# andreaskoepf/faster-rcnn.torch

Hardware: AMD Instinct MI355X
Metric: images/sec (vgg_small 800x450 fwd+bwd) (higher is better)
Workload: dtype f32 (conv / Linear(13824,1024) operands as 2 x fp16 split planes: 22 significand bits, 3 MFMA partial products; fp32 accumulate)

## Files before the change

faster-rcnn.torch_amd/csrc/amax.h:

```cpp
#pragma once
#include <hip/hip_runtime.h>

#include "kernels.h"

namespace frcnn {

__device__ __forceinline__ void amax_store_block(float m, float* rec) {
  __shared__ float amax_part[16];
#pragma unroll
  for (int o = 32; o > 0; o >>= 1) m = fmaxf(m, __shfl_xor(m, o));
  if ((threadIdx.x & 63) == 0) amax_part[threadIdx.x >> 6] = m;
  __syncthreads();
  if (threadIdx.x == 0) {
    const int nw = (blockDim.x + 63) >> 6;
    for (int i = 1; i < nw; ++i) m = fmaxf(m, amax_part[i]);
    rec[1 + blockIdx.x] = m;
    if (blockIdx.x == 0) rec[0] = __builtin_bit_cast(float, (int)gridDim.x);
  }
}

__device__ __forceinline__ float amax_load_block(const float* __restrict__ rec) {
  __shared__ float amax_all[16];
  const int n = __builtin_bit_cast(int, rec[0]);
  float m = 0.f;
  for (int i = threadIdx.x; i < n; i += blockDim.x) m = fmaxf(m, rec[1 + i]);
#pragma unroll
  for (int o = 32; o > 0; o >>= 1) m = fmaxf(m, __shfl_xor(m, o));
  if ((threadIdx.x & 63) == 0) amax_all[threadIdx.x >> 6] = m;
  __syncthreads();
  const int nw = (blockDim.x + 63) >> 6;
  m = amax_all[0];
  for (int i = 1; i < nw; ++i) m = fmaxf(m, amax_all[i]);
  __syncthreads();
  return m;
}

}
```

faster-rcnn.torch_amd/csrc/cnet.hip:

```cpp
#include "kernels.h"

namespace frcnn {

#define BN_EPS 1e-5
#define BN_MOM 0.1

#define BN_CB 16
#define BN_RG 64
template <int CB = BN_CB, int RG = BN_RG>
__device__ __forceinline__ double bn_reduce(double v, double* sh, int tx, int ty) {
  sh[ty * CB + tx] = v;
  __syncthreads();
  for (int stride = RG / 2; stride > 0; stride >>= 1) {
    if (ty < stride) sh[ty * CB + tx] += sh[(ty + stride) * CB + tx];
    __syncthreads();
  }
  const double s = sh[tx];
  __syncthreads();
  return s;
}
template <int NV>
__device__ __forceinline__ void fb_reduce(double (&v)[NV], double* sh, int tx, int ty) {
  const int tid = ty * 4 + tx, lane = tid & 63, wave = tid >> 6;
#pragma unroll
// ... 230 lines not shown
      FR_LAUNCH(KC_ELEMWISE, 0, total * 16.0, s, cnet_act_forward_flat_kernel<true>, dim3(grid), dim3(256), 0, x, src, total, n, lin, slope,
                mask, inv_keep, p, seed, post);
    else
      FR_LAUNCH(KC_ELEMWISE, 0, total * 16.0, s, cnet_act_forward_flat_kernel<false>, dim3(grid), dim3(256), 0, x, src, total, n, lin, slope,
                mask, inv_keep, p, seed, post);
    FR_LAUNCH_CHECK();
    return FRCNN_OK;
  }
  if (gen)
    FR_LAUNCH(KC_ELEMWISE, 0, (double)R * n * 20.0, s, cnet_act_forward_kernel<true>, dim3(cdiv(n, FB_CB)), dim3(FB_CB, FB_RG), 0, x,
              src, R, n, gamma, beta, running, training, lin, xhat, invstd, pre, slope, mask, inv_keep, p, seed, post);
  else
    FR_LAUNCH(KC_ELEMWISE, 0, (double)R * n * 20.0, s, cnet_act_forward_kernel<false>, dim3(cdiv(n, FB_CB)), dim3(FB_CB, FB_RG), 0, x,
              src, R, n, gamma, beta, running, training, lin, xhat, invstd, pre, slope, mask, inv_keep, p, seed, post);
  FR_LAUNCH_CHECK();
  return FRCNN_OK;
}

__global__ __launch_bounds__(1024) void cnet_act_bn_backward_kernel(const float* __restrict__ gy, GemmFold src,
                                                                    const float* __restrict__ pre, const float* __restrict__ xhat,
                                                                    const float* __restrict__ invstd, const float* __restrict__ gamma,
                                                                    const float* slope, const float* __restrict__ mask, float inv_keep,
                                                                    int R, int n, int training, float* __restrict__ gx, float* ggamma,
                                                                    float* gbeta, float* gslope, float* part) {
  __shared__ double sh[FB_RG * FB_CB];
  __shared__ float shs[16];
  const int tx = threadIdx.x, ty = threadIdx.y;
  const int j = blockIdx.x * FB_CB + tx;
  const bool ok = j < n;
  const size_t total = (size_t)R * n;
  const float a = *slope;
  double sg = 0.0, sgx = 0.0;
  float sa = 0.f;
  const bool keep = R <= FB_RG * FB_KEEP;
  float tv[FB_KEEP], xh[FB_KEEP];
  auto first = [&](size_t idx, float& t, float& xhv) {
    float g = fold_value(gy, src, total, idx, j);
    if (mask) g = g * (mask[idx] * inv_keep);
    const float xv = pre[idx];
    t = g;
    if (!(xv > 0.f)) { t = a * g; sa += xv * g; }
    xhv = xhat[idx];
    sg += t;
    sgx += (double)t * xhv;
  };
  if (ok && keep) {
#pragma unroll
// ... 2 lines not shown
      if (ty + i * FB_RG < R) first((size_t)(ty + i * FB_RG) * n + j, tv[i], xh[i]);
    }
  } else if (ok) {
    for (int r = ty; r < R; r += FB_RG) {
      const size_t idx = (size_t)r * n + j;
      float t, xhv;
      first(idx, t, xhv);
      gx[idx] = t;
    }
  }
  { double t[2] = {sg, sgx}; fb_reduce(t, sh, tx, ty); sg = t[0]; sgx = t[1]; }
  {
    const int tid = ty * FB_CB + tx;
#pragma unroll
    for (int o = 32; o > 0; o >>= 1) sa += __shfl_down(sa, o, 64);
    if ((tid & 63) == 0) shs[tid >> 6] = sa;
    __syncthreads();
    if (tid == 0) {
      float t = 0.f;
      for (int i = 0; i < 16; ++i) t += shs[i];
      if (part) part[blockIdx.x] = t; else unsafeAtomicAdd(gslope, t);
    }
  }
  if (!ok) return;
  if (ty == 0) {
    ggamma[j] = (float)((double)ggamma[j] + sgx);
    gbeta[j] = (float)((double)gbeta[j] + sg);
  }
  const double is = invstd[j], gm = gamma[j];
  auto second = [&](size_t idx, double g, double xhv) {
    const double v = training ? (g - sg / R - xhv * sgx / R) * gm * is : g * gm * is;
    gx[idx] = (float)v;
  };
  if (keep) {
#pragma unroll
    for (int i = 0; i < FB_KEEP; ++i)
      if (ty + i * FB_RG < R) second((size_t)(ty + i * FB_RG) * n + j, tv[i], xh[i]);
  } else {
    for (int r = ty; r < R; r += FB_RG) {
      const size_t idx = (size_t)r * n + j;
      second(idx, gx[idx], xhat[idx]);
    }
  }
}
__global__ void slope_fold_kernel(const float* __restrict__ part, int n, float* gslope);
int cnet_act_bn_backward(const float* gy, GemmFold src, const float* pre, const float* xhat, const float* invstd,
                         const float* gamma, const float* slope, const float* mask, float inv_keep, int R, int n, int training,
                         float* gx, float* ggamma, float* gbeta, float* gslope, hipStream_t s) {
  const int grid = cdiv(n, FB_CB);
  float* part = nullptr;
  if (deterministic()) FR_TRY(det_workspace(s, (size_t)grid, &part));
  FR_LAUNCH(KC_ELEMWISE, 0, (double)R * n * 28.0, s, cnet_act_bn_backward_kernel, dim3(grid), dim3(FB_CB, FB_RG), 0, gy, src, pre, xhat,
            invstd, gamma, slope, mask, inv_keep, R, n, training, gx, ggamma, gbeta, gslope, part);
  if (part) FR_LAUNCH(KC_ELEMWISE, 0, grid * 4.0, s, slope_fold_kernel, dim3(1), dim3(1), 0, (const float*)part, grid, gslope);
  FR_LAUNCH_CHECK();
  return FRCNN_OK;
}

template <bool GEN>
__global__ void prelu_dropout_forward_kernel(const float* __restrict__ x, long n, const float* slope,
                                             float* __restrict__ mask, float inv_keep, float p,
                                             unsigned long long seed, float* __restrict__ y) {
  const float a = *slope;
  for (long i = (long)blockIdx.x * blockDim.x + threadIdx.x; i < n; i += (long)gridDim.x * blockDim.x) {
    float v = x[i];
    v = v > 0.f ? v : a * v;
    if (GEN) {
      const float mk = frcnn_keep_mask(seed, (unsigned long long)i, p);
      mask[i] = mk;
      v = v * (mk * inv_keep);
    } else if (mask) {
      v = v * (mask[i] * inv_keep);
    }
    y[i] = v;
  }
}
// ... 340 lines not shown
```

faster-rcnn.torch_amd/csrc/kernels.h:

```cpp
#pragma once
#include <algorithm>

#include "common.h"

namespace frcnn {

int conv_cc(int k);
int conv_mpad(int M);
size_t conv_pack_floats(int Kchan, int M, int k);
int conv_pack_weights(const float* w, int O, int C, int k, float* wf, float* wd, hipStream_t s);
struct PackJob { long w_off; long total; float* dst; int O, C, k, mode, Mpad, blk_begin, nblk; };
PackJob conv_pack_job(long w_off, int O, int C, int k, int mode, float* dst);
int conv_pack_assign_blocks(PackJob* jobs, int njobs, int total_blocks);
int conv_pack_weights_multi(const float* weights, const PackJob* jobs_dev, int njobs, int grid, hipStream_t s);

enum { OUT_STORE = 0, OUT_ADD = 1 };
struct IgemmPool { float* out; unsigned char* idx; const float* slope; const float* scale; float* amax = nullptr; };
int conv_igemm(const float* in, int Cin, int H, int W, const float* in_slope, const float* in_scale,
               const float* wp, const float* bias, int M, int k, int pad, float* out, int out_mode,
               double algo_flops, hipStream_t s, int ws_slot = 0,
               const IgemmPool* pool = nullptr, bool* pool_fused = nullptr);

void set_split_bf16(int on);
int get_split_bf16();
// ... 159 lines not shown
int roi_windows(const double* rect, const long long* pick, int k, const int* layers, int nlayers, int fmH, int fmW, int* wins,
                hipStream_t s);
int detect_post(const int* cls, const float* conf, const float* bbox, const double* rect, const long long* pick, int R,
                int bgclass, double min_conf, float* bb, int* kc, int* keep_row, double* r2, int* K_dev, hipStream_t s);
int detect_gather(const long long* wpick, const int* nwin_dev, int cap, const int* keep_row, const int* kc, const float* bb,
                  const double* r2, const long long* pick, const float* mp, const double* rect, const int* midx, double* rec,
                  hipStream_t s);

int bn_forward(const float* x, int R, int n, const float* gamma, const float* beta, float* running,
               int training, float* xhat, float* invstd, float* y, hipStream_t s);
int bn_backward(const float* gy, const float* xhat, const float* invstd, const float* gamma, int R,
                int n, int training, float* gx, float* ggamma, float* gbeta, hipStream_t s);
int prelu_dropout_forward(const float* x, long n, const float* slope, const float* mask, float inv_keep,
                          float* y, hipStream_t s);
int prelu_dropout_forward_gen(const float* x, long n, const float* slope, float* mask_out, float p,
                              unsigned long long seed, float* y, hipStream_t s);
int prelu_dropout_backward(const float* gy, const float* x, long n, const float* slope,
                           const float* mask, float inv_keep, float* gx, float* gslope, hipStream_t s);
int cnet_act_forward(const float* x, GemmFold src, int R, int n, const float* gamma, const float* beta, float* running,
                     int training, float* lin, float* xhat, float* invstd, float* pre, const float* slope, float* mask, bool gen,
                     float inv_keep, float p, unsigned long long seed, float* post, hipStream_t s);
int cnet_act_bn_backward(const float* gy, GemmFold src, const float* pre, const float* xhat, const float* invstd,
                         const float* gamma, const float* slope, const float* mask, float inv_keep, int R, int n, int training,
                         float* gx, float* ggamma, float* gbeta, float* gslope, hipStream_t s);
bool cnet_heads_fused_eligible(int nf, int nc);
int cnet_heads_forward(const float* x, int R, int nf, const float* Wb, const float* bb, const float* Wc, const float* bc, int nc,
                       float* bbox_out, float* logits, float* lsm, float* cls_out, hipStream_t s);
struct HeadsPostAct {
  const float* pre = nullptr;
  const float* mask = nullptr;
  float inv_keep = 1.f;
  const float* slope = nullptr;
  float* gslope = nullptr;
};
int cnet_heads_backward(const float* g_bbox, const float* g_cls, const float* lsm, int R, int nf, const float* Wb, const float* Wc,
                        int nc, float* glog, float* gfeat, hipStream_t s, const HeadsPostAct* post = nullptr);
int log_softmax_rows_fold(const float* x, GemmFold src, int R, int n, float* y, float* y2, hipStream_t s);
int dropout_mask(float* mask, long n, float p, unsigned long long seed, hipStream_t s);
struct DropoutJobs { float* ptr[8]; int C[8]; float p[8]; unsigned long long seed[8]; int n; };
int dropout_channel_masks(const DropoutJobs& j, hipStream_t s);
int log_softmax_rows(const float* x, int R, int n, float* y, hipStream_t s);
int cnet_losses(float* crout, const float* crtarget, const float* ccout, const float* cctarget, int R,
                int npos, int ncls, float* crdelta, float* ccdelta, double* loss2, hipStream_t s);
int log_softmax_backward(const float* gy, const float* lsm, int R, int n, float* gx, hipStream_t s);
int cnet_decode(const float* cls_lsm, int R, int ncls, int* cls_out, float* conf_out, hipStream_t s);

int image_rgb2yuv(const float* rgb, float* yuv, int H, int W, hipStream_t s);
// ... 16 lines not shown
```

faster-rcnn.torch_amd/csrc/net.cpp:

```cpp
#include <array>
#include <vector>
#include <cmath>
#include <cstring>

#include "kernels.h"

namespace frcnn {

static const int HEAD_OUT = 18;
static const int SPARSE_MAX_POS = 512;

struct DevBuf {
  void* p = nullptr;
  size_t bytes = 0;
  bool owned = true;
  void view(void* ptr, size_t n) { p = ptr; bytes = n; owned = false; }
  int ensure(size_t need) {
    if (need <= bytes) return FRCNN_OK;
    if (p && owned) (void)hipFree(p);
    owned = true;
    p = nullptr; bytes = 0;
    FR_HIP(hipMalloc(&p, need + 64));
    bytes = need;
    return FRCNN_OK;
// ... 36 lines not shown
  DevBuf delta;
  const int* sp_pos = nullptr;
  int sp_count = -1;
  DevBuf spD, spHX, spHY, spGH, spCol, spDX;
  DevBuf spOut, spSlab;
  hipStream_t stream = nullptr;
  hipEvent_t done = nullptr;
  hipEvent_t gin_done = nullptr;
  bool gin_recorded = false;
};

struct ClsLayer {
  int in, n;
  bool bn;
  float p_drop;
  long w_off, b_off, bnw_off, bnb_off, a_off;
  DevBuf lin, pre, post, xhat, invstd, mask, g;
  DevBuf gin;
  DevBuf xp, xpT, gp, gpT;
  int x_form = 0;
  DevBuf am;
  const float* am_w_of = nullptr;
  long am_w_gen = -1;
};

}

using namespace frcnn;

static int g_drop_compact = -1;
static int drop_compact_on() {
  if (g_drop_compact < 0) g_drop_compact = getenv("FRCNN_DROP_COMPACT") ? (atoi(getenv("FRCNN_DROP_COMPACT")) != 0) : 1;
  return g_drop_compact;
}
static int pool_stream(int slot, hipStream_t* out) {
  static hipStream_t pool[8] = {};
  if (!pool[slot]) FR_HIP(hipStreamCreateWithFlags(&pool[slot], hipStreamNonBlocking));
  *out = pool[slot];
  return FRCNN_OK;
}

static int g_sparse_heads = -1;
static int sparse_heads_on() {
  if (g_sparse_heads < 0) g_sparse_heads = getenv("FRCNN_SPARSE_HEADS") ? (atoi(getenv("FRCNN_SPARSE_HEADS")) != 0) : 1;
  return g_sparse_heads;
}
static int g_static_weights = 0;
static long g_static_gen = 0;

struct frcnn_model {
  frcnn_model_desc d;
  std::vector<Conv> convs;
  std::vector<Block> blocks;
  std::vector<Head> heads;
  std::vector<ClsLayer> cls;
  long pnet_params = 0, total_params = 0;
  long bbox_w_off = 0, bbox_b_off = 0, clsw_off = 0, clsb_off = 0;
  int H = 0, W = 0;
  int training = 0;
  DevBuf delta_last;
  DevBuf zero_arena;
  size_t delta_bytes = 0, gpool_bytes = 0;
  DevBuf pack_jobs;
  DevBuf x3_jobs;
  DevBuf amax, amax_ws, amax_jobs;
  int n_amax = 0, n_amax_jobs = 0, amax_grid = 0;
  float* rec(int id) const { return (float*)amax.p + (size_t)id * AMAX_REC; }
  bool f16_packed = false;
  long eval_packs_gen = -1;
  const float* eval_packs_w = nullptr;
  int n_x3_all = 0, n_x3_fwd = 0, x3_grid_all = 0, x3_grid_fwd = 0;
  int n_pack_fwd = 0, n_pack_all = 0, n_pack_heads = 0, pack_grid_fwd = 0, pack_grid_all = 0, pack_grid_heads = 0;
  bool head_packs_fresh = false;
  struct PackGroup { int pk_off = 0, pk_n = 0, pk_grid = 0, am_off = 0, am_n = 0, am_grid = 0, x3_off = 0, x3_off16 = 0, x3_n = 0, x3_grid = 0; };
  std::vector<PackGroup> groups;
  unsigned fresh_mask = 0;
  const float* fresh_w = nullptr;
  bool fresh_f16 = false;
  static const int DC_RING = 4;
  char* dc_pin = nullptr; DevBuf dc_dev; size_t dc_slot_bytes = 0, dc_idx_off = 0; unsigned dc_step = 0;
  hipEvent_t dc_ev[DC_RING] = {};
  std::vector<PackXJob> x3_host, x3_host16;
  std::vector<int> x3_conv;
  DevBuf dbg_expand;
  std::vector<hipEvent_t> block_rd_ev;
  hipStream_t side = nullptr;
  hipStream_t cw = nullptr;
  hipEvent_t cw_fork = nullptr, cw_done = nullptr;
  bool cw_pending = false;
  std::vector<hipEvent_t> cw_ev;
// ... 235 lines not shown
      }
      m->pk_bb_off = (int)both.size(); m->pk_bb_n = (int)gj.size();
      m->pk_bb_grid = gj.empty() ? 0 : conv_pack_assign_blocks(gj.data(), m->pk_bb_n, 512);
      both.insert(both.end(), gj.begin(), gj.end());
    }
    FR_TRY(m->pack_jobs.ensure(both.size() * sizeof(PackJob)));
    FR_HIP(hipMemcpy(m->pack_jobs.p, both.data(), both.size() * sizeof(PackJob), hipMemcpyHostToDevice));
  }
  {
    {
      int n = 0;
      for (auto& c : m->convs) { c.am = n; n += 3; }
      for (auto& hd : m->heads) { hd.c3.am = n; n += 3; }
      for (auto& b : m->blocks) b.am = n++;
      m->n_amax = n;
      FR_TRY(m->amax.ensure((size_t)n * AMAX_REC * 4));
      FR_TRY(m->amax_ws.ensure((size_t)n * 4));
      std::vector<AmaxJob> aj;
      auto addw = [&](Conv& c) {
        if (c.x_f || c.x_d) aj.push_back(AmaxJob{c.w_off, (long)c.Cout * c.Cin * c.k * c.k, m->rec(c.am + 2), 0});
      };
      for (auto& c : m->convs) addw(c);
      for (auto& hd : m->heads) addw(hd.c3);
      m->n_amax_jobs = (int)aj.size();
      m->amax_grid = tensor_absmax_assign_blocks(aj.data(), m->n_amax_jobs);
      FR_CHECK(m->amax_grid >= 0, "ensure_shapes: a weight tensor is too large for its magnitude record");
      {
        std::vector<AmaxJob> gj;
        for (auto& c : m->convs)
          if (c.x_f || c.x_d) gj.push_back(AmaxJob{c.w_off, (long)c.Cout * c.Cin * c.k * c.k, m->rec(c.am + 2), 0});
        m->am_bb_off = (int)aj.size(); m->am_bb_n = (int)gj.size();
        m->am_bb_grid = gj.empty() ? 0 : tensor_absmax_assign_blocks(gj.data(), m->am_bb_n);
        aj.insert(aj.end(), gj.begin(), gj.end());
      }
      for (size_t g = 0; g <= m->blocks.size(); ++g) {
        std::vector<AmaxJob> gj;
        auto addg = [&](Conv& c) {
          if (c.x_f || c.x_d) gj.push_back(AmaxJob{c.w_off, (long)c.Cout * c.Cin * c.k * c.k, m->rec(c.am + 2), 0});
        };
        if (g < m->blocks.size()) { for (auto& c : m->convs) if (c.block == (int)g) addg(c); }
        else for (auto& hd : m->heads) addg(hd.c3);
        auto& G = m->groups[g];
        G.am_off = (int)aj.size(); G.am_n = (int)gj.size();
        G.am_grid = gj.empty() ? 0 : tensor_absmax_assign_blocks(gj.data(), G.am_n);
        FR_CHECK(G.am_grid >= 0, "ensure_shapes: a weight tensor is too large for its magnitude record");
        aj.insert(aj.end(), gj.begin(), gj.end());
      }
      if (!aj.empty()) {
        FR_TRY(m->amax_jobs.ensure(aj.size() * sizeof(AmaxJob)));
        FR_HIP(hipMemcpy(m->amax_jobs.p, aj.data(), aj.size() * sizeof(AmaxJob), hipMemcpyHostToDevice));
      }
    }
    std::vector<PackXJob> all, fwd, all16, fwd16;
// ... 94 lines not shown
  frcnn_model* m = new frcnn_model();
  m->d = *desc;
  build_layout(m);
  *out = m;
  return FRCNN_OK;
}

int frcnn_model_destroy(frcnn_model* m) {
  if (!m) return FRCNN_OK;
  auto rel = [](Conv& c) { c.wf.release(); c.wd.release(); c.wx.release(); c.wxd.release(); c.x.release(); c.gx.release(); };
  for (auto& c : m->convs) rel(c);
  for (auto& b : m->blocks) { b.scale.release(); b.pooled.release(); b.gpooled.release(); b.pidx.release(); b.dc_bias.release(); }
  if (m->dc_pin) (void)hipHostFree(m->dc_pin);
  for (auto e : m->dc_ev) if (e) (void)hipEventDestroy(e);
  m->dc_dev.release(); m->dbg_expand.release();
  for (auto& h : m->heads) {
    rel(h.c3); rel(h.c1); h.delta.release(); h.spOut.release(); h.spSlab.release();
    h.spD.release(); h.spHX.release(); h.spHY.release(); h.spGH.release(); h.spCol.release(); h.spDX.release();
  }
  for (auto& l : m->cls) {
    l.lin.release(); l.pre.release(); l.post.release(); l.xhat.release(); l.invstd.release();
    l.mask.release(); l.g.release(); l.xp.release(); l.xpT.release(); l.gp.release(); l.gpT.release(); l.am.release();
  }
  m->img.release(); m->wg_ws.release(); m->wg_ws_first.release(); m->pack_jobs.release(); m->x3_jobs.release(); m->zero_arena.release(); m->amax.release(); m->amax_ws.release(); m->amax_jobs.release();
  for (auto e : m->fork_ev) (void)hipEventDestroy(e);
  for (auto& h : m->heads) {
    if (h.done) (void)hipEventDestroy(h.done);
    if (h.gin_done) (void)hipEventDestroy(h.gin_done);
  }
  if (m->chain_ev) (void)hipEventDestroy(m->chain_ev);
  if (m->join_ev) (void)hipEventDestroy(m->join_ev);
  if (m->bwd_ev) (void)hipEventDestroy(m->bwd_ev);
  if (m->heads_gin_ev) (void)hipEventDestroy(m->heads_gin_ev);
  if (m->upd_ev) (void)hipEventDestroy(m->upd_ev);
  if (m->upd_join_ev) (void)hipEventDestroy(m->upd_join_ev);
  for (auto e : m->block_rd_ev) (void)hipEventDestroy(e);
  for (auto e : m->cw_ev) (void)hipEventDestroy(e);
  if (m->cw_fork) (void)hipEventDestroy(m->cw_fork);
  if (m->cw_done) (void)hipEventDestroy(m->cw_done);
  if (m->loss_ev) (void)hipEventDestroy(m->loss_ev);
  for (auto e : m->block_ev) (void)hipEventDestroy(e);
  m->delta_last.release(); m->feat_g.release(); m->logits.release(); m->lsm.release(); m->glog.release();
  m->gtmp.release();
  delete m;
  return FRCNN_OK;
}

// ... 304 lines not shown
  async_heads = async_heads && use_side && training;
  m->heads_deferred = async_heads && sparse_heads_on() && !deterministic() && m->heads.size() <= 4;
  m->heads_sparse_fwd = false; m->heads_gin = false;
  m->last_w = w;
  if (use_side && !m->heads_deferred) { FR_TRY(ensure_side(m)); FR_TRY(ensure_head_streams(m)); }
  DropoutJobs dj;
  dj.n = 0;
  for (size_t b = 0; b < m->blocks.size(); ++b) {
    Block& blk = m->blocks[b];
    if (!blk.has_drop) continue;
    int C = m->d.filters[b];
    if (!training) {
      FR_TRY(fill_value(blk.scale.f(), C, 1.0f - blk.p_drop, s));
    } else if (drop_masks && drop_masks[b]) {
      FR_HIP(hipMemcpyAsync(blk.scale.p, drop_masks[b], (size_t)C * 4, hipMemcpyDeviceToDevice, s));
    } else {
      dj.ptr[dj.n] = blk.scale.f(); dj.C[dj.n] = C; dj.p[dj.n] = blk.p_drop; dj.seed[dj.n] = seed * 131 + b;
      ++dj.n;
    }
  }
  FR_TRY(dropout_channel_masks(dj, s));
  FR_TRY(plan_compact(m, training, drop_masks, seed));
  m->head_packs_fresh = false;
  const bool f16 = get_x3_f16() && m->n_amax_jobs > 0;
  const bool reuse = !training && g_static_weights && m->eval_packs_gen == g_static_gen && m->eval_packs_w == w && m->f16_packed == f16;
  m->f16_packed = f16;
  const bool fresh = training && !m->groups.empty() && m->fresh_mask == (1u << m->groups.size()) - 1 && m->fresh_w == w && m->fresh_f16 == f16 &&
                     !any_compact(m);
  m->fresh_mask = 0;
  if (!reuse && !fresh) {
    static const bool skip_on = !(getenv("FRCNN_HEAD_PACK_SKIP") && atoi(getenv("FRCNN_HEAD_PACK_SKIP")) == 0);
    const bool skip_heads = skip_on && training && m->heads_deferred && any_compact(m) && m->am_bb_n > 0;
    m->head_x3_fresh = !skip_heads;
    if (training && skip_heads) {
      if (m->pk_bb_n) FR_TRY(conv_pack_weights_multi(w, (const PackJob*)m->pack_jobs.p + m->pk_bb_off, m->pk_bb_n, m->pk_bb_grid, s));
    } else if (training)
      FR_TRY(conv_pack_weights_multi(w, (const PackJob*)m->pack_jobs.p, m->n_pack_all, m->pack_grid_all, s));
    else
      FR_TRY(conv_pack_weights_multi(w, (const PackJob*)m->pack_jobs.p + m->n_pack_all, m->n_pack_fwd, m->pack_grid_fwd, s));
    const PackXJob* xjobs = (const PackXJob*)m->x3_jobs.p + (f16 ? m->n_x3_all + m->n_x3_fwd : 0);
    if (f16 && skip_heads)
      FR_TRY(tensor_absmax_multi(w, (const AmaxJob*)m->amax_jobs.p + m->am_bb_off, m->am_bb_n, m->am_bb_grid, s));
    else if (f16)
      FR_TRY(tensor_absmax_multi(w, (const AmaxJob*)m->amax_jobs.p, m->n_amax_jobs, m->amax_grid, s));
    if (training && any_compact(m))
      FR_TRY(pack_compact(m, w, f16, s));
    else if (training)
      FR_TRY(conv_x3_pack_multi(w, xjobs, m->n_x3_all, m->x3_grid_all, s));
    else
      FR_TRY(conv_x3_pack_multi(w, xjobs + m->n_x3_all, m->n_x3_fwd, m->x3_grid_fwd, s));
  }
  m->eval_packs_gen = training ? -1 : g_static_gen;
  m->eval_packs_w = w;
  FR_TRY(m->img.ensure((size_t)3 * H * W * 4));
  FR_HIP(hipMemcpyAsync(m->img.p, img, (size_t)3 * H * W * 4, hipMemcpyDeviceToDevice, s));
  const float* cur = m->img.f();
  const float* cur_slope = nullptr;
  const float* cur_scale = nullptr;
  const float* cur_am = nullptr;
  for (size_t b = 0; b < m->blocks.size(); ++b) {
    Block& blk = m->blocks[b];
    bool pooled_in_conv = false;
    for (int st = 0; st < blk.nconv; ++st) {
      Conv& c = m->convs[blk.first_conv + st];
      const bool last = st == blk.nconv - 1;
      IgemmPool pl = {blk.pooled.f(), (unsigned char*)blk.pidx.p, w + c.a_off,
                      (st == 0 && blk.has_drop) ? blk.scale.f() : nullptr, f16 ? m->rec(blk.am) : nullptr};
// ... 100 lines not shown
    } break;
    case 4: {
      FR_CHECK(index >= 0 && index < (int)m->blocks.size() && m->H > 0 && m->blocks[index].has_drop, "debug_buffer: block %d has no dropout", index);
      const Block& k = m->blocks[index]; b = &k.scale; n = (size_t)m->d.filters[index] * 4;
    } break;
    case 1: {
      FR_CHECK(index >= 0 && index < (int)m->blocks.size() && m->H > 0, "debug_buffer: block %d (after a forward pass)", index);
      const Block& k = m->blocks[index]; b = &k.pidx; n = (size_t)m->d.filters[index] * k.Hp * k.Wp;
    } break;
    case 2: {
      FR_CHECK(index >= 0 && index < (int)m->heads.size() && m->H > 0, "debug_buffer: anchor net %d (after a forward pass)", index);
      const Conv& c = m->heads[index].c3; b = &c.x; n = (size_t)c.Cout * c.Ho * c.Wo * 4;
      if ((m->heads_sparse_fwd || m->heads_deferred) && m->last_w) {
        FR_HIP(hipDeviceSynchronize());
        if (!m->head_x3_fresh) { FR_TRY(refresh_group(m, m->last_w, (int)m->blocks.size(), nullptr)); m->head_x3_fresh = true; }
        FR_TRY(head_forward(m, m->heads[index], m->last_w, nullptr, 0));
        FR_HIP(hipDeviceSynchronize());
      }
    } break;
    case 3: {
      FR_CHECK(index >= 0 && index < (int)m->cls.size() && m->R > 0, "debug_buffer: classification layer %d (after frcnn_cnet_forward)", index);
      const ClsLayer& L = m->cls[index]; b = L.bn ? &L.pre : &L.lin; n = (size_t)m->R * L.n * 4;
    } break;
    default: FR_CHECK(false, "debug_buffer: unknown kind %d", kind);
  }
  FR_CHECK(b->p && b->bytes >= n, "debug_buffer: buffer not allocated yet");
  *ptr = b->p; *bytes = (long long)n;
  return FRCNN_OK;
}

int frcnn_pnet_delta(frcnn_model* m, int i, float** ptr) {
  FR_CHECK(m->H > 0, "pnet_delta: call frcnn_pnet_forward first");
  FR_CHECK(i >= 1 && i <= (int)m->heads.size() + 1, "pnet_delta: index %d out of range", i);
  *ptr = i <= (int)m->heads.size() ? m->heads[i - 1].delta.f() : m->delta_last.f();
  return FRCNN_OK;
}

int frcnn_pnet_set_sparse_deltas(frcnn_model* m, int head, const int* positions, int count) {
  FR_CHECK(head >= 1 && head <= (int)m->heads.size(), "pnet_set_sparse_deltas: head %d out of range", head);
  m->heads[head - 1].sp_pos = positions;
  m->heads[head - 1].sp_count = count;
  return FRCNN_OK;
}

int frcnn_pnet_zero_deltas(frcnn_model* m, void* stream) {
  FR_CHECK(m->H > 0, "pnet_zero_deltas: call frcnn_pnet_forward first");
// ... 288 lines not shown
}

int frcnn_pnet_wait_heads_done(frcnn_model* m, void* stream) {
  FR_CHECK(m->block_ev_valid, "pnet_wait_heads_done: call frcnn_pnet_backward first");
  for (auto& h : m->heads)
    if (h.stream && h.done) FR_HIP(hipStreamWaitEvent(S(stream), h.done, 0));
  if (m->side) {
    FR_TRY(ensure_update_stream(m));
    FR_TRY(chain(m->side, S(stream), m->upd_ev));
  }
  return FRCNN_OK;
}

int frcnn_pnet_wait_block_done(frcnn_model* m, int block, void* stream) {
  FR_CHECK(block >= 1 && block <= (int)m->blocks.size(), "pnet_wait_block_done: block %d out of range", block);
  FR_CHECK(m->update_armed && m->block_ev_valid && (size_t)block <= m->block_ev.size() && (size_t)block <= m->block_rd_ev.size(),
           "pnet_wait_block_done: call frcnn_model_update_stream before the pass and frcnn_pnet_backward first");
  FR_HIP(hipStreamWaitEvent(S(stream), m->block_ev[block - 1], 0));
  FR_HIP(hipStreamWaitEvent(S(stream), m->block_rd_ev[block - 1], 0));
  return FRCNN_OK;
}

static int refresh_group(frcnn_model* m, const float* w, int group, hipStream_t s) {
  const bool f16 = get_x3_f16() && m->n_amax_jobs > 0;
  const frcnn_model::PackGroup& G = m->groups[group];
  if (G.pk_n) FR_TRY(conv_pack_weights_multi(w, (const PackJob*)m->pack_jobs.p + G.pk_off, G.pk_n, G.pk_grid, s));
  if (f16 && G.am_n) FR_TRY(tensor_absmax_multi(w, (const AmaxJob*)m->amax_jobs.p + G.am_off, G.am_n, G.am_grid, s));
  if (G.x3_n) FR_TRY(conv_x3_pack_multi(w, (const PackXJob*)m->x3_jobs.p + (f16 ? G.x3_off16 : G.x3_off), G.x3_n, G.x3_grid, s));
  return FRCNN_OK;
}
int frcnn_pnet_refresh_packs(frcnn_model* m, const float* w, int group, void* stream) {
  FR_CHECK(m->H > 0, "pnet_refresh_packs: call frcnn_pnet_forward first");
  FR_CHECK(group >= 0 && group < (int)m->groups.size(), "pnet_refresh_packs: group %d out of range", group);
  const bool f16 = get_x3_f16() && m->n_amax_jobs > 0;
  if (m->fresh_mask && (m->fresh_w != w || m->fresh_f16 != f16)) m->fresh_mask = 0;
  FR_TRY(refresh_group(m, w, group, S(stream)));
  if (group == (int)m->blocks.size()) m->head_x3_fresh = true;
  m->fresh_mask |= 1u << group; m->fresh_w = w; m->fresh_f16 = f16;
  return FRCNN_OK;
}

int frcnn_pnet_invalidate_packs(frcnn_model* m) {
  m->fresh_mask = 0;
  return FRCNN_OK;
}

int frcnn_pnet_wait_block_gradients(frcnn_model* m, int block, void* stream) {
  FR_CHECK(block >= 1 && block <= (int)m->blocks.size(), "pnet_wait_block_gradients: block %d out of range", block);
  FR_CHECK(m->block_ev_valid && (size_t)block <= m->block_ev.size(), "pnet_wait_block_gradients: call frcnn_pnet_backward first");
  FR_HIP(hipStreamWaitEvent(S(stream), m->block_ev[block - 1], 0));
  return FRCNN_OK;
}

static int record_block_read(frcnn_model* m, int b, hipStream_t s) {
  if (!m->update_armed) return FRCNN_OK;
  while (m->block_rd_ev.size() < m->blocks.size()) {
    hipEvent_t e;
// ... 189 lines not shown
    if (L.x_form & 1) FR_TRY(L.xp.ensure((size_t)3 * R * L.in * 2));
    if (L.x_form & 2) FR_TRY(L.gp.ensure((size_t)3 * R * L.n * 2));
    if (L.x_form & 4) { FR_TRY(L.xpT.ensure((size_t)3 * L.in * Rp * 2)); FR_TRY(L.gpT.ensure((size_t)3 * L.n * Rp * 2)); }
    if (L.x_form & 7) FR_TRY(L.am.ensure((size_t)5 * AMAX_REC * 4));
  }
  int nc = m->d.class_count + 1;
  int nf = m->cls.empty() ? m->D : m->cls.back().n;
  FR_TRY(m->feat_g.ensure((size_t)R * nf * 4));
  FR_TRY(m->logits.ensure((size_t)R * nc * 4));
  FR_TRY(m->lsm.ensure((size_t)R * nc * 4));
  FR_TRY(m->glog.ensure((size_t)R * nc * 4));
  return FRCNN_OK;
}

int frcnn_cnet_forward(frcnn_model* m, const float* weights, const float* x, int R, int training,
                       const float* const* drop_masks, unsigned long long seed, float* bn_running,
                       float* bbox_out, float* cls_out, void* stream) {
  hipStream_t s = S(stream);
  FR_CHECK(R > 0, "cnet_forward: empty batch");
  FR_TRY(cw_join(m, s));
  FR_TRY(ensure_cnet(m, R));
  m->R = R; m->cnet_x = x; m->training = training;
  const float* w = weights;
  const float* cur = x;
  float* bnr = bn_running;
  for (size_t l = 0; l < m->cls.size(); ++l) {
    ClsLayer& L = m->cls[l];
    GemmFold fold;
    GemmFold* defer = cnet_fuse() ? &fold : nullptr;
    if ((L.x_form & 3) && gemm_f16_on()) {
      float* rw = L.am.f() + 2 * AMAX_REC;
      const bool have = !training && g_static_weights && L.am_w_gen == g_static_gen && L.am_w_of == w;
      if (!have) FR_TRY(tensor_absmax(w + L.w_off, (long)L.n * L.in, rw, s));
      L.am_w_of = w; L.am_w_gen = training ? -1 : g_static_gen;
    } else {
      L.am_w_of = nullptr;
    }
    if ((L.x_form & 1) && gemm_f16_on()) {
      float* rx = L.am.f();
      FR_TRY(tensor_absmax(cur, (long)R * L.in, rx, s));
      FR_TRY(split_planes(cur, R, L.in, L.xp.p, nullptr, s, rx));
      FR_TRY(linear_x_forward(L.xp.p, R, L.in, w + L.w_off, w + L.b_off, L.n, L.lin.f(), s, 0, defer, rx, rx + 2 * AMAX_REC));
    } else if (L.x_form & 1) {
      FR_TRY(split_planes(cur, R, L.in, L.xp.p, nullptr, s));
      FR_TRY(linear_x_forward(L.xp.p, R, L.in, w + L.w_off, w + L.b_off, L.n, L.lin.f(), s, 0, defer));
    } else {
      FR_TRY(gemm_f32(cur, L.in, 1, w + L.w_off, 1, L.in, L.lin.f(), L.n, R, L.n, L.in, OUT_STORE, w + L.b_off, s, 0, defer));
    }
    if (L.bn) FR_CHECK(training || bnr, "cnet_forward: evaluate mode needs bn_running");
    const float* mask = nullptr;
    float inv_keep = 1.f;
    bool draw = false;
    if (training && L.p_drop > 0.f) {
      inv_keep = 1.0f / (1.0f - L.p_drop);
      if (drop_masks && drop_masks[l])
        FR_HIP(hipMemcpyAsync(L.mask.p, drop_masks[l], (size_t)R * L.n * 4, hipMemcpyDeviceToDevice, s));
      else
        draw = true;
      mask = L.mask.f();
    }
    if (defer) {
      FR_TRY(cnet_act_forward(L.lin.f(), fold, R, L.n, L.bn ? w + L.bnw_off : nullptr, L.bn ? w + L.bnb_off : nullptr, L.bn ? bnr : nullptr,
                              training, L.lin.f(), L.xhat.f(), L.invstd.f(), L.pre.f(), w + L.a_off, const_cast<float*>(mask), draw,
                              inv_keep, L.p_drop, seed * 977 + l + 17, L.post.f(), s));
      if (L.bn && bnr) bnr += 2 * L.n;
// ... 74 lines not shown
      post.slope = w + T.a_off; post.gslope = grad + T.a_off;
      dst = T.g.f();
      top_act_done = true;
    }
    FR_TRY(cnet_heads_backward(g_bbox, g_cls, m->lsm.f(), R, nf, w + m->bbox_w_off, w + m->clsw_off, nc, m->glog.f(), dst, s,
                               top_act_done ? &post : nullptr));
    FR_TRY(fork());
  } else {
    FR_TRY(log_softmax_backward(g_cls, m->lsm.f(), R, nc, m->glog.f(), s));
    FR_TRY(fork());
    FR_TRY(gemm_f32(g_bbox, 4, 1, w + m->bbox_w_off, nf, 1, m->feat_g.f(), nf, R, nf, 4, OUT_STORE, nullptr, s));
    FR_TRY(gemm_f32(m->glog.f(), nc, 1, w + m->clsw_off, nf, 1, m->feat_g.f(), nf, R, nf, nc, OUT_ADD, nullptr, s));
  }
  FR_TRY(gemm_f32(g_bbox, 1, 4, feat, nf, 1, grad + m->bbox_w_off, nf, 4, nf, R, OUT_ADD, nullptr, ws, wslot));
  FR_TRY(channel_sum_cols(g_bbox, R, 4, grad + m->bbox_b_off, ws));
  FR_TRY(gemm_f32(m->glog.f(), 1, nc, feat, nf, 1, grad + m->clsw_off, nf, nc, nf, R, OUT_ADD, nullptr, ws, wslot));
  FR_TRY(channel_sum_cols(m->glog.f(), R, nc, grad + m->clsb_off, ws));
  const float* g = m->feat_g.f();
  GemmFold gfold;
  for (int l = (int)m->cls.size() - 1; l >= 0; --l) {
    ClsLayer& L = m->cls[l];
    const float* pre = L.bn ? L.pre.f() : L.lin.f();
    const bool drop = m->training && L.p_drop > 0.f;
    if (top_act_done && l == (int)m->cls.size() - 1) {
    } else if (L.bn && cnet_fuse()) {
      FR_TRY(cnet_act_bn_backward(g, gfold, pre, L.xhat.f(), L.invstd.f(), w + L.bnw_off, w + L.a_off, drop ? L.mask.f() : nullptr,
                                  drop ? 1.0f / (1.0f - L.p_drop) : 1.f, R, L.n, m->training, L.g.f(), grad + L.bnw_off,
                                  grad + L.bnb_off, grad + L.a_off, s));
    } else {
      FR_TRY(prelu_dropout_backward(g, pre, (long)R * L.n, w + L.a_off, drop ? L.mask.f() : nullptr,
                                    drop ? 1.0f / (1.0f - L.p_drop) : 1.f, L.g.f(), grad + L.a_off, s));
      if (L.bn)
        FR_TRY(bn_backward(L.g.f(), L.xhat.f(), L.invstd.f(), w + L.bnw_off, R, L.n, m->training, L.g.f(),
                           grad + L.bnw_off, grad + L.bnb_off, s));
    }
    gfold = GemmFold{};
    GemmFold* gdefer = (cnet_fuse() && async && l > 0 && m->cls[l - 1].bn) ? &gfold : nullptr;
    FR_TRY(fork());
    const float* in = l == 0 ? m->cnet_x : m->cls[l - 1].post.f();
    float* gin = l == 0 ? gx : L.gin.f();
    const bool xw = (L.x_form & 4) != 0, xd = (L.x_form & 2) != 0 && gin;
    if (xd && gemm_f16_on() && L.am_w_of == w) {
      float* rg = L.am.f() + AMAX_REC;
      FR_TRY(tensor_absmax(L.g.f(), (long)R * L.n, rg, s));
      FR_TRY(split_planes(L.g.f(), R, L.n, L.gp.p, nullptr, s, rg));
      FR_TRY(linear_x_dgrad(L.gp.p, R, L.n, w + L.w_off, L.in, gin, OUT_STORE, s, 0, gdefer, rg, L.am.f() + 2 * AMAX_REC));
    } else if (xd) {
      FR_TRY(split_planes(L.g.f(), R, L.n, L.gp.p, nullptr, s));
      FR_TRY(linear_x_dgrad(L.gp.p, R, L.n, w + L.w_off, L.in, gin, OUT_STORE, s, 0, gdefer));
    } else if (gin) {
      FR_TRY(gemm_f32(L.g.f(), L.n, 1, w + L.w_off, L.in, 1, gin, L.in, R, L.in, L.n, OUT_STORE, nullptr, s, 0, gdefer));
    }
    static const bool wgrad_f16 = !(getenv("FRCNN_GEMM_WGRAD_F16") && atoi(getenv("FRCNN_GEMM_WGRAD_F16")) == 0);
    if (xw && wgrad_f16 && gemm_f16_on() && L.am.bytes >= (size_t)5 * AMAX_REC * 4) {
      float *rgT = L.am.f() + 3 * AMAX_REC, *rxT = L.am.f() + 4 * AMAX_REC;
      FR_TRY(tensor_absmax(L.g.f(), (long)R * L.n, rgT, ws));
      if ((L.x_form & 1) && L.am_w_of == w) rxT = L.am.f();
      else FR_TRY(tensor_absmax(in, (long)R * L.in, rxT, ws));
      FR_TRY(split_planes(L.g.f(), R, L.n, nullptr, L.gpT.p, ws, rgT));
      FR_TRY(split_planes(in, R, L.in, nullptr, L.xpT.p, ws, rxT));
      FR_TRY(linear_x_wgrad(L.gpT.p, L.xpT.p, R, L.n, L.in, grad + L.w_off, ws, wslot, rgT, rxT));
    } else if (xw) {
      FR_TRY(split_planes(L.g.f(), R, L.n, nullptr, L.gpT.p, ws));
      FR_TRY(split_planes(in, R, L.in, nullptr, L.xpT.p, ws));
      FR_TRY(linear_x_wgrad(L.gpT.p, L.xpT.p, R, L.n, L.in, grad + L.w_off, ws, wslot));
    } else {
      FR_TRY(gemm_f32(L.g.f(), 1, L.n, in, L.in, 1, grad + L.w_off, L.in, L.n, L.in, R, OUT_ADD, nullptr, ws, wslot));
    }
    FR_TRY(channel_sum_cols(L.g.f(), R, L.n, grad + L.b_off, ws));
    g = gin;
  }
  if (m->cls.empty() && gx) FR_HIP(hipMemcpyAsync(gx, g, (size_t)R * m->D * 4, hipMemcpyDeviceToDevice, s));
  if (async) {
    FR_HIP(hipEventRecord(m->cw_done, ws));
    m->cw_pending = true;
  }
  return FRCNN_OK;
}

// ... 2 lines not shown
```

Measured before the change: 515.7.

## Fuse gradient absmax into BN backward and batch cnet weight absmax with pack jobs

The fused activation/BN backward kernel now also records each block's gradient magnitude maximum. The separate tensor_absmax passes on the classifier gradient (for dgrad and wgrad) can then be dropped, and the wgrad path reuses that record. Classifier weight absmax jobs are appended to the existing multi-tensor absmax launch at the start of a step, so the forward pass can skip its per-layer weight absmax launches. This saves several small kernel launches and extra reads of the gradient and weights, at the cost of more bookkeeping state and a cross-stream dependency on the head-of-step record.

```diff
diff --git a/faster-rcnn.torch_amd/csrc/amax.h b/faster-rcnn.torch_amd/csrc/amax.h
--- a/faster-rcnn.torch_amd/csrc/amax.h
+++ b/faster-rcnn.torch_amd/csrc/amax.h
@@ -5,19 +5,20 @@
 
 namespace frcnn {
 
-__device__ __forceinline__ void amax_store_block(float m, float* rec) {
+__device__ __forceinline__ void amax_store_block(float m, float* rec, int tid, int nthreads) {
   __shared__ float amax_part[16];
 #pragma unroll
   for (int o = 32; o > 0; o >>= 1) m = fmaxf(m, __shfl_xor(m, o));
-  if ((threadIdx.x & 63) == 0) amax_part[threadIdx.x >> 6] = m;
+  if ((tid & 63) == 0) amax_part[tid >> 6] = m;
   __syncthreads();
-  if (threadIdx.x == 0) {
-    const int nw = (blockDim.x + 63) >> 6;
+  if (tid == 0) {
+    const int nw = (nthreads + 63) >> 6;
     for (int i = 1; i < nw; ++i) m = fmaxf(m, amax_part[i]);
     rec[1 + blockIdx.x] = m;
     if (blockIdx.x == 0) rec[0] = __builtin_bit_cast(float, (int)gridDim.x);
   }
 }
+__device__ __forceinline__ void amax_store_block(float m, float* rec) { amax_store_block(m, rec, threadIdx.x, blockDim.x); }
 
 __device__ __forceinline__ float amax_load_block(const float* __restrict__ rec) {
   __shared__ float amax_all[16];
diff --git a/faster-rcnn.torch_amd/csrc/cnet.hip b/faster-rcnn.torch_amd/csrc/cnet.hip
--- a/faster-rcnn.torch_amd/csrc/cnet.hip
+++ b/faster-rcnn.torch_amd/csrc/cnet.hip
@@ -1,3 +1,4 @@
+#include "amax.h"
 #include "kernels.h"
 
 namespace frcnn {
@@ -276,7 +277,7 @@
                                                                     const float* __restrict__ invstd, const float* __restrict__ gamma,
                                                                     const float* slope, const float* __restrict__ mask, float inv_keep,
                                                                     int R, int n, int training, float* __restrict__ gx, float* ggamma,
-                                                                    float* gbeta, float* gslope, float* part) {
+                                                                    float* gbeta, float* gslope, float* part, float* amax_rec) {
   __shared__ double sh[FB_RG * FB_CB];
   __shared__ float shs[16];
   const int tx = threadIdx.x, ty = threadIdx.y;
@@ -325,36 +326,41 @@
       if (part) part[blockIdx.x] = t; else unsafeAtomicAdd(gslope, t);
     }
   }
-  if (!ok) return;
-  if (ty == 0) {
-    ggamma[j] = (float)((double)ggamma[j] + sgx);
-    gbeta[j] = (float)((double)gbeta[j] + sg);
-  }
-  const double is = invstd[j], gm = gamma[j];
-  auto second = [&](size_t idx, double g, double xhv) {
-    const double v = training ? (g - sg / R - xhv * sgx / R) * gm * is : g * gm * is;
-    gx[idx] = (float)v;
-  };
-  if (keep) {
-#pragma unroll
-    for (int i = 0; i < FB_KEEP; ++i)
-      if (ty + i * FB_RG < R) second((size_t)(ty + i * FB_RG) * n + j, tv[i], xh[i]);
-  } else {
-    for (int r = ty; r < R; r += FB_RG) {
-      const size_t idx = (size_t)r * n + j;
-      second(idx, gx[idx], xhat[idx]);
-    }
-  }
+  float am = 0.f;
+  if (ok) {
+    if (ty == 0) {
+      ggamma[j] = (float)((double)ggamma[j] + sgx);
+      gbeta[j] = (float)((double)gbeta[j] + sg);
+    }
+    const double is = invstd[j], gm = gamma[j];
+    auto second = [&](size_t idx, double g, double xhv) {
+      const double v = training ? (g - sg / R - xhv * sgx / R) * gm * is : g * gm * is;
+      gx[idx] = (float)v;
+      am = fmaxf(am, fabsf((float)v));
+    };
+    if (keep) {
+#pragma unroll
+      for (int i = 0; i < FB_KEEP; ++i)
+        if (ty + i * FB_RG < R) second((size_t)(ty + i * FB_RG) * n + j, tv[i], xh[i]);
+    } else {
+      for (int r = ty; r < R; r += FB_RG) {
+        const size_t idx = (size_t)r * n + j;
+        second(idx, gx[idx], xhat[idx]);
+      }
+    }
+  }
+  if (amax_rec) amax_store_block(am, amax_rec, ty * FB_CB + tx, FB_CB * FB_RG);
 }
 __global__ void slope_fold_kernel(const float* __restrict__ part, int n, float* gslope);
 int cnet_act_bn_backward(const float* gy, GemmFold src, const float* pre, const float* xhat, const float* invstd,
                          const float* gamma, const float* slope, const float* mask, float inv_keep, int R, int n, int training,
-                         float* gx, float* ggamma, float* gbeta, float* gslope, hipStream_t s) {
+                         float* gx, float* ggamma, float* gbeta, float* gslope, hipStream_t s, float* amax_rec) {
   const int grid = cdiv(n, FB_CB);
+  FR_CHECK(!amax_rec || grid <= AMAX_MAX_BLOCKS, "cnet_act_bn_backward: %d blocks, more than a magnitude record holds", grid);
   float* part = nullptr;
   if (deterministic()) FR_TRY(det_workspace(s, (size_t)grid, &part));
   FR_LAUNCH(KC_ELEMWISE, 0, (double)R * n * 28.0, s, cnet_act_bn_backward_kernel, dim3(grid), dim3(FB_CB, FB_RG), 0, gy, src, pre, xhat,
-            invstd, gamma, slope, mask, inv_keep, R, n, training, gx, ggamma, gbeta, gslope, part);
+            invstd, gamma, slope, mask, inv_keep, R, n, training, gx, ggamma, gbeta, gslope, part, amax_rec);
   if (part) FR_LAUNCH(KC_ELEMWISE, 0, grid * 4.0, s, slope_fold_kernel, dim3(1), dim3(1), 0, (const float*)part, grid, gslope);
   FR_LAUNCH_CHECK();
   return FRCNN_OK;
diff --git a/faster-rcnn.torch_amd/csrc/kernels.h b/faster-rcnn.torch_amd/csrc/kernels.h
--- a/faster-rcnn.torch_amd/csrc/kernels.h
+++ b/faster-rcnn.torch_amd/csrc/kernels.h
@@ -205,7 +205,7 @@
                      float inv_keep, float p, unsigned long long seed, float* post, hipStream_t s);
 int cnet_act_bn_backward(const float* gy, GemmFold src, const float* pre, const float* xhat, const float* invstd,
                          const float* gamma, const float* slope, const float* mask, float inv_keep, int R, int n, int training,
-                         float* gx, float* ggamma, float* gbeta, float* gslope, hipStream_t s);
+                         float* gx, float* ggamma, float* gbeta, float* gslope, hipStream_t s, float* amax_rec = nullptr);
 bool cnet_heads_fused_eligible(int nf, int nc);
 int cnet_heads_forward(const float* x, int R, int nf, const float* Wb, const float* bb, const float* Wc, const float* bc, int nc,
                        float* bbox_out, float* logits, float* lsm, float* cls_out, hipStream_t s);
diff --git a/faster-rcnn.torch_amd/csrc/net.cpp b/faster-rcnn.torch_amd/csrc/net.cpp
--- a/faster-rcnn.torch_amd/csrc/net.cpp
+++ b/faster-rcnn.torch_amd/csrc/net.cpp
@@ -82,6 +82,7 @@
   DevBuf am;
   const float* am_w_of = nullptr;
   long am_w_gen = -1;
+  const float* am_w_rec = nullptr;
 };
 
 }
@@ -104,6 +105,14 @@
 static int sparse_heads_on() {
   if (g_sparse_heads < 0) g_sparse_heads = getenv("FRCNN_SPARSE_HEADS") ? (atoi(getenv("FRCNN_SPARSE_HEADS")) != 0) : 1;
   return g_sparse_heads;
+}
+static bool cnet_wrec_on() {
+  static const bool on = !(getenv("FRCNN_CNET_WREC") && atoi(getenv("FRCNN_CNET_WREC")) == 0);
+  return on;
+}
+static bool cnet_grec_on() {
+  static const bool on = !(getenv("FRCNN_CNET_GREC") && atoi(getenv("FRCNN_CNET_GREC")) == 0);
+  return on;
 }
 static int g_static_weights = 0;
 static long g_static_gen = 0;
@@ -126,6 +135,10 @@
   DevBuf amax, amax_ws, amax_jobs;
   int n_amax = 0, n_amax_jobs = 0, amax_grid = 0;
   float* rec(int id) const { return (float*)amax.p + (size_t)id * AMAX_REC; }
+  DevBuf cls_amw;
+  int n_amax_cnet = 0;
+  const float* cls_amw_of = nullptr;
+  hipStream_t cls_amw_s = nullptr;
   bool f16_packed = false;
   long eval_packs_gen = -1;
   const float* eval_packs_w = nullptr;
@@ -407,6 +420,14 @@
       };
       for (auto& c : m->convs) addw(c);
       for (auto& hd : m->heads) addw(hd.c3);
+      std::vector<AmaxJob> cj;
+      if (cnet_wrec_on() && !m->cls.empty()) {
+        FR_TRY(m->cls_amw.ensure(m->cls.size() * AMAX_REC * 4));
+        for (size_t l = 0; l < m->cls.size(); ++l)
+          cj.push_back(AmaxJob{m->cls[l].w_off, (long)m->cls[l].n * m->cls[l].in, m->cls_amw.f() + l * AMAX_REC, 0});
+      }
+      aj.insert(aj.end(), cj.begin(), cj.end());
+      m->n_amax_cnet = (int)cj.size();
       m->n_amax_jobs = (int)aj.size();
       m->amax_grid = tensor_absmax_assign_blocks(aj.data(), m->n_amax_jobs);
       FR_CHECK(m->amax_grid >= 0, "ensure_shapes: a weight tensor is too large for its magnitude record");
@@ -414,6 +435,7 @@
         std::vector<AmaxJob> gj;
         for (auto& c : m->convs)
           if (c.x_f || c.x_d) gj.push_back(AmaxJob{c.w_off, (long)c.Cout * c.Cin * c.k * c.k, m->rec(c.am + 2), 0});
+        gj.insert(gj.end(), cj.begin(), cj.end());
         m->am_bb_off = (int)aj.size(); m->am_bb_n = (int)gj.size();
         m->am_bb_grid = gj.empty() ? 0 : tensor_absmax_assign_blocks(gj.data(), m->am_bb_n);
         aj.insert(aj.end(), gj.begin(), gj.end());
@@ -554,7 +576,7 @@
     l.lin.release(); l.pre.release(); l.post.release(); l.xhat.release(); l.invstd.release();
     l.mask.release(); l.g.release(); l.xp.release(); l.xpT.release(); l.gp.release(); l.gpT.release(); l.am.release();
   }
-  m->img.release(); m->wg_ws.release(); m->wg_ws_first.release(); m->pack_jobs.release(); m->x3_jobs.release(); m->zero_arena.release(); m->amax.release(); m->amax_ws.release(); m->amax_jobs.release();
+  m->cls_amw.release(); m->img.release(); m->wg_ws.release(); m->wg_ws_first.release(); m->pack_jobs.release(); m->x3_jobs.release(); m->zero_arena.release(); m->amax.release(); m->amax_ws.release(); m->amax_jobs.release();
   for (auto e : m->fork_ev) (void)hipEventDestroy(e);
   for (auto& h : m->heads) {
     if (h.done) (void)hipEventDestroy(h.done);
@@ -905,15 +927,16 @@
   FR_TRY(dropout_channel_masks(dj, s));
   FR_TRY(plan_compact(m, training, drop_masks, seed));
   m->head_packs_fresh = false;
-  const bool f16 = get_x3_f16() && m->n_amax_jobs > 0;
+  const bool f16 = get_x3_f16() && m->n_amax_jobs > m->n_amax_cnet;
   const bool reuse = !training && g_static_weights && m->eval_packs_gen == g_static_gen && m->eval_packs_w == w && m->f16_packed == f16;
   m->f16_packed = f16;
   const bool fresh = training && !m->groups.empty() && m->fresh_mask == (1u << m->groups.size()) - 1 && m->fresh_w == w && m->fresh_f16 == f16 &&
                      !any_compact(m);
   m->fresh_mask = 0;
+  m->cls_amw_of = nullptr;
   if (!reuse && !fresh) {
     static const bool skip_on = !(getenv("FRCNN_HEAD_PACK_SKIP") && atoi(getenv("FRCNN_HEAD_PACK_SKIP")) == 0);
-    const bool skip_heads = skip_on && training && m->heads_deferred && any_compact(m) && m->am_bb_n > 0;
+    const bool skip_heads = skip_on && training && m->heads_deferred && any_compact(m) && m->am_bb_n > m->n_amax_cnet;
     m->head_x3_fresh = !skip_heads;
     if (training && skip_heads) {
       if (m->pk_bb_n) FR_TRY(conv_pack_weights_multi(w, (const PackJob*)m->pack_jobs.p + m->pk_bb_off, m->pk_bb_n, m->pk_bb_grid, s));
@@ -926,6 +949,7 @@
       FR_TRY(tensor_absmax_multi(w, (const AmaxJob*)m->amax_jobs.p + m->am_bb_off, m->am_bb_n, m->am_bb_grid, s));
     else if (f16)
       FR_TRY(tensor_absmax_multi(w, (const AmaxJob*)m->amax_jobs.p, m->n_amax_jobs, m->amax_grid, s));
+    if (f16 && training && m->cls_amw.p) { m->cls_amw_of = w; m->cls_amw_s = s; }
     if (training && any_compact(m))
       FR_TRY(pack_compact(m, w, f16, s));
     else if (training)
@@ -1072,6 +1096,17 @@
       FR_CHECK(index >= 0 && index < (int)m->cls.size() && m->R > 0, "debug_buffer: classification layer %d (after frcnn_cnet_forward)", index);
       const ClsLayer& L = m->cls[index]; b = L.bn ? &L.pre : &L.lin; n = (size_t)m->R * L.n * 4;
     } break;
+    case 5: {
+      FR_CHECK(index >= 0 && index / 4 < (int)m->cls.size(), "debug_buffer: classification layer %d", index / 4);
+      const ClsLayer& L = m->cls[index / 4];
+      const int which = index % 4;
+      n = (size_t)AMAX_REC * 4;
+      if (which < 2) { FR_CHECK(L.am.p, "debug_buffer: layer %d keeps no records", index / 4); *ptr = L.am.f() + which * AMAX_REC; }
+      else if (which == 2) { FR_CHECK(L.am_w_rec, "debug_buffer: the last forward pass used no weight record"); *ptr = (void*)L.am_w_rec; }
+      else { FR_CHECK(m->cls_amw.p, "debug_buffer: no head-of-step weight records"); *ptr = m->cls_amw.f() + (index / 4) * AMAX_REC; }
+      *bytes = (long long)n;
+      return FRCNN_OK;
+    }
     default: FR_CHECK(false, "debug_buffer: unknown kind %d", kind);
   }
   FR_CHECK(b->p && b->bytes >= n, "debug_buffer: buffer not allocated yet");
@@ -1406,7 +1441,7 @@
 }
 
 static int refresh_group(frcnn_model* m, const float* w, int group, hipStream_t s) {
-  const bool f16 = get_x3_f16() && m->n_amax_jobs > 0;
+  const bool f16 = get_x3_f16() && m->n_amax_jobs > m->n_amax_cnet;
   const frcnn_model::PackGroup& G = m->groups[group];
   if (G.pk_n) FR_TRY(conv_pack_weights_multi(w, (const PackJob*)m->pack_jobs.p + G.pk_off, G.pk_n, G.pk_grid, s));
   if (f16 && G.am_n) FR_TRY(tensor_absmax_multi(w, (const AmaxJob*)m->amax_jobs.p + G.am_off, G.am_n, G.am_grid, s));
@@ -1416,7 +1451,7 @@
 int frcnn_pnet_refresh_packs(frcnn_model* m, const float* w, int group, void* stream) {
   FR_CHECK(m->H > 0, "pnet_refresh_packs: call frcnn_pnet_forward first");
   FR_CHECK(group >= 0 && group < (int)m->groups.size(), "pnet_refresh_packs: group %d out of range", group);
-  const bool f16 = get_x3_f16() && m->n_amax_jobs > 0;
+  const bool f16 = get_x3_f16() && m->n_amax_jobs > m->n_amax_cnet;
   if (m->fresh_mask && (m->fresh_w != w || m->fresh_f16 != f16)) m->fresh_mask = 0;
   FR_TRY(refresh_group(m, w, group, S(stream)));
   if (group == (int)m->blocks.size()) m->head_x3_fresh = true;
@@ -1652,6 +1687,8 @@
   FR_TRY(ensure_cnet(m, R));
   m->R = R; m->cnet_x = x; m->training = training;
   const float* w = weights;
+  const bool head_wrec = training && m->cls_amw_of == w && m->cls_amw_s == s;
+  m->cls_amw_of = nullptr;
   const float* cur = x;
   float* bnr = bn_running;
   for (size_t l = 0; l < m->cls.size(); ++l) {
@@ -1661,16 +1698,17 @@
     if ((L.x_form & 3) && gemm_f16_on()) {
       float* rw = L.am.f() + 2 * AMAX_REC;
       const bool have = !training && g_static_weights && L.am_w_gen == g_static_gen && L.am_w_of == w;
-      if (!have) FR_TRY(tensor_absmax(w + L.w_off, (long)L.n * L.in, rw, s));
-      L.am_w_of = w; L.am_w_gen = training ? -1 : g_static_gen;
+      if (head_wrec) rw = m->cls_amw.f() + l * AMAX_REC;
+      else if (!have) FR_TRY(tensor_absmax(w + L.w_off, (long)L.n * L.in, rw, s));
+      L.am_w_of = w; L.am_w_gen = training ? -1 : g_static_gen; L.am_w_rec = rw;
     } else {
-      L.am_w_of = nullptr;
+      L.am_w_of = nullptr; L.am_w_rec = nullptr;
     }
     if ((L.x_form & 1) && gemm_f16_on()) {
       float* rx = L.am.f();
       FR_TRY(tensor_absmax(cur, (long)R * L.in, rx, s));
       FR_TRY(split_planes(cur, R, L.in, L.xp.p, nullptr, s, rx));
-      FR_TRY(linear_x_forward(L.xp.p, R, L.in, w + L.w_off, w + L.b_off, L.n, L.lin.f(), s, 0, defer, rx, rx + 2 * AMAX_REC));
+      FR_TRY(linear_x_forward(L.xp.p, R, L.in, w + L.w_off, w + L.b_off, L.n, L.lin.f(), s, 0, defer, rx, L.am_w_rec));
     } else if (L.x_form & 1) {
       FR_TRY(split_planes(cur, R, L.in, L.xp.p, nullptr, s));
       FR_TRY(linear_x_forward(L.xp.p, R, L.in, w + L.w_off, w + L.b_off, L.n, L.lin.f(), s, 0, defer));
@@ -1791,11 +1829,14 @@
     ClsLayer& L = m->cls[l];
     const float* pre = L.bn ? L.pre.f() : L.lin.f();
     const bool drop = m->training && L.p_drop > 0.f;
+    const bool grec_want = cnet_grec_on() && gemm_f16_on() && (L.x_form & 6) && L.am.bytes >= (size_t)5 * AMAX_REC * 4;
+    float* grec = nullptr;
     if (top_act_done && l == (int)m->cls.size() - 1) {
     } else if (L.bn && cnet_fuse()) {
+      if (grec_want) grec = L.am.f() + AMAX_REC;
       FR_TRY(cnet_act_bn_backward(g, gfold, pre, L.xhat.f(), L.invstd.f(), w + L.bnw_off, w + L.a_off, drop ? L.mask.f() : nullptr,
                                   drop ? 1.0f / (1.0f - L.p_drop) : 1.f, R, L.n, m->training, L.g.f(), grad + L.bnw_off,
-                                  grad + L.bnb_off, grad + L.a_off, s));
+                                  grad + L.bnb_off, grad + L.a_off, s, grec));
     } else {
       FR_TRY(prelu_dropout_backward(g, pre, (long)R * L.n, w + L.a_off, drop ? L.mask.f() : nullptr,
                                     drop ? 1.0f / (1.0f - L.p_drop) : 1.f, L.g.f(), grad + L.a_off, s));
@@ -1811,9 +1852,9 @@
     const bool xw = (L.x_form & 4) != 0, xd = (L.x_form & 2) != 0 && gin;
     if (xd && gemm_f16_on() && L.am_w_of == w) {
       float* rg = L.am.f() + AMAX_REC;
-      FR_TRY(tensor_absmax(L.g.f(), (long)R * L.n, rg, s));
+      if (!grec) FR_TRY(tensor_absmax(L.g.f(), (long)R * L.n, rg, s));
       FR_TRY(split_planes(L.g.f(), R, L.n, L.gp.p, nullptr, s, rg));
-      FR_TRY(linear_x_dgrad(L.gp.p, R, L.n, w + L.w_off, L.in, gin, OUT_STORE, s, 0, gdefer, rg, L.am.f() + 2 * AMAX_REC));
+      FR_TRY(linear_x_dgrad(L.gp.p, R, L.n, w + L.w_off, L.in, gin, OUT_STORE, s, 0, gdefer, rg, L.am_w_rec));
     } else if (xd) {
       FR_TRY(split_planes(L.g.f(), R, L.n, L.gp.p, nullptr, s));
       FR_TRY(linear_x_dgrad(L.gp.p, R, L.n, w + L.w_off, L.in, gin, OUT_STORE, s, 0, gdefer));
@@ -1823,7 +1864,8 @@
     static const bool wgrad_f16 = !(getenv("FRCNN_GEMM_WGRAD_F16") && atoi(getenv("FRCNN_GEMM_WGRAD_F16")) == 0);
     if (xw && wgrad_f16 && gemm_f16_on() && L.am.bytes >= (size_t)5 * AMAX_REC * 4) {
       float *rgT = L.am.f() + 3 * AMAX_REC, *rxT = L.am.f() + 4 * AMAX_REC;
-      FR_TRY(tensor_absmax(L.g.f(), (long)R * L.n, rgT, ws));
+      if (grec) rgT = grec;
+      else FR_TRY(tensor_absmax(L.g.f(), (long)R * L.n, rgT, ws));
       if ((L.x_form & 1) && L.am_w_of == w) rxT = L.am.f();
       else FR_TRY(tensor_absmax(in, (long)R * L.in, rxT, ws));
       FR_TRY(split_planes(L.g.f(), R, L.n, nullptr, L.gpT.p, ws, rgT));
```

Result: no change. 514.9, median of 6 (-0.2%).
